# microsoft/Cream

Measured on AMD Instinct MI355X. Metric: images/sec (whole node) AutoFormer-S supernet step @224^2, higher is better.
Workload: dtype bf16; 1 GPU; AutoFormer-S supernet train step, random-path sampling (random.seed(epoch)), per-GPU batch 128, 224x224, AdamW, grad all-reduce RCCL; global_batch=128, parallelism=dp1, wgrad_partials=bf16 split-K partial tiles (within 1.9e-3 of fp32 partials), mixup=on-device, in the timed region

## Files before the change

### cream_amd/_lib.py

```python
import ctypes
import os

_HERE = os.path.dirname(os.path.abspath(__file__))
LIB_PATH = os.path.join(_HERE, "libcream_amd.so")

CREAM_OK = 0
_ERRORS = {
    -1: "CREAM_ERR_BAD_ARG (null pointer, negative size or unsupported stride)",
    -2: "CREAM_ERR_BAD_DTYPE (element type not supported by this entry point)",
    -3: "CREAM_ERR_LAUNCH (HIP kernel launch failed)",
    -4: "CREAM_ERR_TOO_LARGE (shape exceeds what the kernel family supports)",
}

F32, F16, BF16, F64 = 0, 1, 2, 3


class CreamLibraryError(RuntimeError):
    pass


_c = ctypes
_vp, _i, _i64, _f = _c.c_void_p, _c.c_int, _c.c_int64, _c.c_float

SIGNATURES = {
# ... 18 lines not shown
    "cream_irpe_attn2_check": (_i, [_vp, _i]),
    "cream_irpe_attn2_fwd": (_i, [_vp, _vp]),
    "cream_irpe_attn2_bwd": (_i, [_vp, _vp]),
    "cream_irpe_table_grad2": (_i, [_vp, _vp, _i64, _i64, _i64, _i, _vp, _i64, _i64, _i64, _i, _i, _i, _i, _f, _vp]),
    "cream_mini_attn_fwd": (_i, [_vp, _vp]),
    "cream_mini_attn_bwd": (_i, [_vp, _vp]),
    "cream_window_attn_check": (_i, [_vp, _i]),
    "cream_window_attn_part_size": (_i, [_i, _i, _i]),
    "cream_window_attn_blocks": (_i, [_vp]),
    "cream_window_attn_fwd": (_i, [_vp, _vp]),
    "cream_window_attn_bwd": (_i, [_vp, _vp]),
    "cream_window_attn_large_check": (_i, [_vp, _i]),
    "cream_window_attn_large_part_size": (_i, [_i, _i]),
    "cream_window_attn_large_blocks": (_i, [_vp]),
    "cream_window_attn_large_fwd": (_i, [_vp, _vp]),
    "cream_window_attn_large_bwd": (_i, [_vp, _vp]),
    "cream_token_dwconv3_part_size": (_i, [_i]),
    "cream_token_dwconv3_blocks": (_i, [_vp]),
    "cream_token_dwconv3_fwd": (_i, [_vp, _vp]),
    "cream_token_dwconv3_bwd": (_i, [_vp, _vp]),
    "cream_cga_attn_check": (_i, [_vp]),
    "cream_cga_attn_fwd": (_i, [_vp, _vp]),
    "cream_relation_loss_check": (_i, [_vp]),
    "cream_relation_loss_blocks": (_i, [_vp]),
    "cream_relation_loss": (_i, [_vp, _vp]),
    "cream_hidden_relation_check": (_i, [_vp]),
    "cream_hidden_relation_padded": (_i, [_i]),
    "cream_hidden_relation_parts": (_i, [_i, _i]),
    "cream_hidden_relation_loss": (_i, [_vp, _vp]),
    "cream_attn_rpe2d_padded_len": (_i, [_i]),
    "cream_attn_rpe2d_dtab_parts": (_i, [_i, _i]),
    "cream_attn_rpe2d_bwd_mode": (_i, [_i]),
    "cream_attn_rpe2d_fwd": (_i, [_vp, _vp, _vp, _vp, _vp, _vp, _i64, _i64, _i64, _vp, _vp, _vp, _vp, _i,
                                  _i, _i, _i, _i, _i, _i, _f, _i, _vp]),
    "cream_attn_rpe2d_bwd": (_i, [_vp, _vp, _vp, _i64, _i64, _i64, _vp, _vp, _vp, _vp, _vp,
                                  _vp, _vp, _vp, _vp, _vp, _vp, _vp, _i64, _i64, _i64,
                                  _vp, _vp, _vp, _vp, _i, _i, _i, _i, _i, _i, _i, _f, _i, _vp]),
    "cream_attn_rpe2d_fwd_img": (_i, [_vp, _vp, _vp, _vp, _vp, _vp, _i64, _i64, _i64, _vp, _vp, _vp, _vp, _i, _vp,
                                      _i, _i, _i, _i, _i, _i, _f, _i, _vp]),
    "cream_attn_rpe2d_bwd_img": (_i, [_vp, _vp, _vp, _i64, _i64, _i64, _vp, _vp, _vp, _vp, _vp,
                                      _vp, _vp, _vp, _vp, _vp, _vp, _vp, _i64, _i64, _i64,
                                      _vp, _vp, _vp, _vp, _i, _vp, _i, _i, _i, _i, _i, _i, _f, _i, _vp]),
    "cream_attn_rpe2d_fwd_drop": (_i, [_vp, _vp, _vp, _vp, _vp, _vp, _i64, _i64, _i64, _vp, _vp, _vp, _vp, _i, _vp,
                                       _i, _i, _i, _i, _i, _i, _f, _f, _c.c_uint32, _i, _vp]),
    "cream_attn_rpe2d_bwd_drop": (_i, [_vp, _vp, _vp, _i64, _i64, _i64, _vp, _vp, _vp, _vp, _vp,
                                       _vp, _vp, _vp, _vp, _vp, _vp, _vp, _i64, _i64, _i64,
                                       _vp, _vp, _vp, _vp, _i, _vp, _i, _i, _i, _i, _i, _i, _f, _f, _c.c_uint32, _i, _vp]),
    "cream_attn_rpe2d_table_image_bytes": (_i64, []),
    "cream_attn_rpe2d_table_images": (_i, [_vp, _vp, _vp, _vp, _vp, _i, _i, _vp]),
    "cream_attn_rpe2d_fwd_mode": (_i, [_i]),
    "cream_ln_fwd": (_i, [_vp, _vp, _vp, _vp, _vp, _vp, _i, _i, _f, _vp]),
    "cream_ln_partials": (_i, []),
    "cream_ln_bwd": (_i, [_vp, _vp, _vp, _vp, _vp, _vp, _vp, _vp, _vp, _vp, _i, _i, _i, _vp]),
    "cream_gelu_fwd": (_i, [_vp, _vp, _i64, _vp]),
    "cream_gelu_bwd": (_i, [_vp, _vp, _vp, _i64, _vp]),
    "cream_residual_add": (_i, [_vp, _vp, _vp, _vp, _i64, _i64, _vp]),
    "cream_scale_cast": (_i, [_vp, _vp, _vp, _i64, _i64, _vp]),
    "cream_colsum_slabs": (_i, [_i]),
    "cream_colsum": (_i, [_vp, _vp, _i, _i, _vp]),
    "cream_add_ln_fwd": (_i, [_vp, _vp, _vp, _vp, _vp, _vp, _vp, _i, _vp, _vp, _i, _i, _f, _vp]),
    "cream_block_wgrad_bf16": (_i, [_i]),
    "cream_colsum128_slabs": (_i, [_i]),
    "cream_colsum128": (_i, [_vp, _vp, _i, _i, _vp]),
    "cream_gelu_bwd_colsum": (_i, [_vp, _vp, _vp, _vp, _i, _i, _vp]),
    "cream_scale_cast_colsum": (_i, [_vp, _vp, _vp, _vp, _i, _i, _i, _vp]),
    "cream_grad_finalize": (_i, [_vp, _i, _vp]),
    "cream_gemm_rows_per_colsum_slab": (_i, []),
    "cream_gemm_nt256": (_i, [_i]),
    "cream_gemm_nt8": (_i, [_i]),
    "cream_linear_fwd": (_i, [_vp, _vp, _vp, _vp, _i, _i, _i, _i64, _vp]),
    "cream_linear_fwd_seg": (_i, [_vp, _vp, _vp, _vp, _i, _i, _i, _i64, _i, _i64, _vp]),
    "cream_linear_gelu_fwd": (_i, [_vp, _vp, _vp, _vp, _vp, _i, _i, _i, _i64, _vp]),
    "cream_linear_gelu_fwd_pad": (_i, [_vp, _vp, _vp, _vp, _vp, _i, _i, _i, _i, _i64, _vp]),
    "cream_linear_dgrad": (_i, [_vp, _vp, _vp, _i, _i, _i, _i64, _vp]),
    "cream_linear_dgrad_seg": (_i, [_vp, _vp, _vp, _i, _i, _i, _i64, _i, _i64, _vp]),
    "cream_linear_dgrad_mul": (_i, [_vp, _vp, _vp, _vp, _vp, _i, _i, _i, _i64, _vp]),
    "cream_linear_wgrad_splits": (_i, [_i, _i, _i]),
    "cream_linear_wgrad_splits_bf16": (_i, [_i, _i, _i]),
    "cream_gemm_tn8": (_i, [_i]),
    "cream_gemm_nthalf": (_i, [_i]),
    "cream_gemm_nt224": (_i, [_i]),
    "cream_gemm_nt224_launches": (_i64, []),
    "cream_linear_nt224": (_i, [_vp, _vp, _vp, _vp, _i, _i, _i, _i64, _i, _i64, _i, _i64, _vp]),
    "cream_gemm_ntopt": (_i, [_i]),
    "cream_gemm_stagger": (_i, [_i]),
    "cream_block_layout_epoch": (_i, []),
    "cream_cu_reserve": (_i, [_i]),
    "cream_mixup_cutmix": (_i, [_vp, _vp, _vp, _i, _i, _i, _i, _i, _f, _i, _i, _i, _i, _i, _f, _vp]),
    "cream_image_batch_plan": (_i64, [_vp, _i, _i, _i]),
    "cream_image_batch_transform": (_i, [_vp, _vp, _i64, _vp, _vp, _i, _i, _i, _vp, _vp, _vp, _i64, _vp]),
    "cream_cu_count": (_i, []),
    "cream_linear_wgrad_parts": (_i, [_vp, _vp, _vp, _vp, _i, _i, _i, _i, _vp]),
    "cream_linear_wgrad_parts_bf16": (_i, [_vp, _vp, _vp, _vp, _i, _i, _i, _i, _vp]),
    "cream_param_job_tiles": (_i, [_i, _i]),
    "cream_adamw_step": (_i, [_vp, _vp, _i, _i, _i, _c.c_double, _c.c_double, _c.c_double, _c.c_double, _i64, _vp]),
    "cream_grad_clip_coef": (_i, [_vp, _vp, _i, _i, _c.c_double, _vp, _vp, _vp]),
    "cream_adamw_step_clipped": (_i, [_vp, _vp, _i, _i, _i, _c.c_double, _c.c_double, _c.c_double, _c.c_double, _i64, _vp, _vp]),
    "cream_grad_scale": (_i, [_vp, _vp, _i, _i, _vp, _vp]),
    "cream_soft_ce": (_i, [_vp, _vp, _vp, _vp, _i, _i, _i, _f, _vp]),
    "cream_sparse_ce": (_i, [_vp, _vp, _vp, _vp, _vp, _i, _i, _i, _i, _f, _vp]),
    "cream_softmax_topk_records": (_i, [_vp, _vp, _vp, _i, _i, _i, _i, _vp]),
    "cream_linear_f32_fwd": (_i, [_vp, _vp, _vp, _vp, _i, _i, _i, _i64, _i64, _i, _i, _vp]),
    "cream_bmm_f32": (_i, [_vp, _vp, _vp, _i, _i, _i, _vp, _vp, _vp, _i, _i, _vp]),
    "cream_linear_f32_dgrad": (_i, [_vp, _vp, _vp, _i, _i, _i, _i64, _i, _i, _vp]),
    "cream_linear_f32_wgrad": (_i, [_vp, _vp, _vp, _vp, _i, _i, _i, _i64, _i64, _i, _i, _vp]),
    "cream_ln_f32_fwd": (_i, [_vp, _vp, _vp, _vp, _vp, _vp, _i, _i, _f, _vp]),
    "cream_ln_f32_bwd": (_i, [_vp, _vp, _vp, _vp, _vp, _vp, _vp, _i, _i, _vp]),
    "cream_block_prof_enable": (_i, [_i]),
    "cream_block_prof_kinds": (_i, []),
    "cream_block_prof_name": (_c.c_char_p, [_i]),
    "cream_block_prof_collect": (_i, [_vp, _vp, _vp, _vp]),
    "cream_slices_copy": (_i, [_vp, _i, _vp, _i, _i, _vp]),
    "cream_block_fwd_workspace": (_i64, [_vp, _vp, _vp, _vp]),
    "cream_block_fwd": (_i, [_vp, _vp, _vp, _vp, _vp, _vp, _vp]),
    "cream_block_bwd_workspace": (_i64, [_vp, _vp, _vp, _vp]),
    "cream_block_bwd": (_i, [_vp, _vp, _vp, _vp, _vp, _vp, _vp, _vp, _i, _i64, _vp, _vp, _i, _vp, _vp]),
    "cream_image_augment_workspace": (_i64, [_i, _i, _i, _i]),
    "cream_image_augment_u8": (_i, [_vp, _vp, _i, _i, _i, _vp, _vp, _i, _vp, _i64, _vp]),
    "cream_image_batch_plan_aug": (_i64, [_vp, _i, _i, _i, _vp, _i]),
    "cream_image_batch_transform_aug": (_i, [_vp, _vp, _i64, _vp, _vp, _i, _i, _i, _vp, _vp, _vp, _vp, _i, _vp, _i64, _vp]),
}

MAX_GRAD_JOBS = 24


class GradJob(ctypes.Structure):
    _fields_ = [("dst", _vp), ("src", _vp), ("ld", _i64), ("pstride", _i64),
                ("nparts", _c.c_int32), ("rows", _c.c_int32), ("cols", _c.c_int32),
                ("interleave", _c.c_int32), ("src_bf16", _c.c_int32), ("overwrite", _c.c_int32)]

class ImageDesc(ctypes.Structure):
    _fields_ = ([("offset", _i64)] +
                [(n, _c.c_int32) for n in ("height", "width", "row_stride", "box_top", "box_left", "box_h", "box_w", "resized_h",
                                           "resized_w", "win_top", "win_left", "flip", "row0", "nrows")] +
                [("tmp_off", _i64)] +
                [(n, _c.c_int32) for n in ("erase_top", "erase_left", "erase_h", "erase_w")] +
                [("erase_seed", _c.c_uint32), ("reserved", _c.c_int32)])


class AugOp(ctypes.Structure):
    _fields_ = [("kind", _c.c_int32), ("arg", _c.c_int32), ("factor", _f), ("fill", _c.c_uint32), ("m", _c.c_double * 6)]


class SliceJob(ctypes.Structure):
    _fields_ = [("full", _vp), ("ld", _i64), ("packed_off", _i64), ("rows", _c.c_int32), ("cols", _c.c_int32)]


class BlockDesc(ctypes.Structure):
    _fields_ = ([(n, _c.c_int32) for n in ("B", "N", "E", "H", "F", "gh", "gw", "mr", "F_valid", "inference")] +
                [(n, _f) for n in ("eps1", "eps2", "attn_scale", "reserved_f")] +
                [(n, _vp) for n in ("wqkv", "wqkv_t", "bqkv", "wproj", "wproj_t", "bproj", "w1", "w1_t", "b1",
                                    "w2", "w2_t", "b2")] +
                [(n, _i64) for n in ("ld_qkv", "ld_qkv_t", "seg_qkv", "seg_qkv_t", "ld_proj", "ld_proj_t", "ld_w1",
                                     "ld_w1_t", "ld_w2", "ld_w2_t")] +
                [(n, _vp) for n in ("ln1_g", "ln1_b", "ln2_g", "ln2_b", "tkv", "tkh", "tvv", "tvh")] +
                [("ldt", _i64), ("timg", _vp)])


class IrpeAttnDesc(ctypes.Structure):
    _fields_ = ([(n, _vp) for n in ("q", "k", "v")] + [(n, _i64) for n in ("sb", "sn", "sh")] +
                [(n, _vp) for n in ("out", "lse", "sv", "wq", "wk", "wv")] +
                [(n, _i64) for n in ("wq_hs", "wk_hs", "wv_hs")] +
                [(n, _vp) for n in ("idq", "idk", "idv", "idq_t", "idk_t", "idv_t")] +
                [(n, _c.c_int32) for n in ("B", "H", "L", "NP", "nb")] + [("scale", _f)] +
                [(n, _vp) for n in ("dout", "dq", "dk", "dv")] + [(n, _i64) for n in ("dsb", "dsn", "dsh")] +
                [(n, _vp) for n in ("delta", "lkg", "gg", "dlk", "dlq", "bq", "bk")] + [(n, _i64) for n in ("bq_hs", "bk_hs")] +
# ... 128 lines not shown
```

### cream_amd/csrc/gemm_mfma.hip

```cpp
#include <hip/hip_runtime.h>
#include <stdint.h>
#include <stdlib.h>
#include <atomic>

#include "cream_amd.h"
#include "gemm_mfma.hpp"
#include "gemm_nt8.hpp"
#include "gemm_nt224.hpp"
#include "gemm_tn8.hpp"
#include "launch_ev.hpp"
#include "cu_budget.hpp"
#include "env_switch.hpp"

namespace {
std::atomic<int> g_cu_reserve{0};
std::atomic<int> g_layout_epoch{0};
int physical_cus()
{
    static int cus = 0;
    if (!cus) {
        int dev = 0;
        hipDeviceProp_t prop;
        if (hipGetDevice(&dev) == hipSuccess && hipGetDeviceProperties(&prop, dev) == hipSuccess) cus = prop.multiProcessorCount;
        if (cus <= 0) cus = 256;
    }
    return cus;
}
}
namespace cream {
int cu_count()
{
    int c = (physical_cus() - g_cu_reserve.load(std::memory_order_relaxed)) / 8 * 8;
    return c < 8 ? 8 : c;
}
}

namespace {
using namespace cream;
using namespace cream::gemm;

int num_cus() { return cream::cu_count(); }

EnvSwitch g_nt256{"CREAM_GEMM_NT256", 2};
int nt256_mode() { return g_nt256.get(); }

EnvSwitch g_ntopt{"CREAM_GEMM_NTOPT", 3, [](int m) { return m & 15; }};
int ntopt_mode() { return g_ntopt.get(); }
EnvSwitch g_stagger{"CREAM_GEMM_STAGGER", 0};
int stagger_mode() { return g_stagger.get(); }

template <int EPI>
int launch_nt256(const NtParams& p, hipStream_t st)
{
    constexpr int BM = 256, BN = 256;
    auto kern = (ntopt_mode() & 4) ? gemm_nt_kernel<BM, BN, 2, 4, 2, EPI, 1, 1> : gemm_nt_kernel<BM, BN, 2, 4, 2, EPI, 1>;
    constexpr int lds = nt_lds_bytes(BM, BN, 2);
    if (!cream::raise_dynamic_lds(kern, lds)) return CREAM_ERR_LAUNCH;
    const int tiles = ((p.M + BM - 1) / BM) * ((p.N + BN - 1) / BN), slots = num_cus() / 8 * 8;
    CREAM_LAUNCH(kern, dim3(tiles < slots ? tiles : slots), dim3(512), lds, st, p);
    return hipGetLastError() == hipSuccess ? CREAM_OK : CREAM_ERR_LAUNCH;
}

EnvSwitch g_nt8{"CREAM_GEMM_NT8", 4};
int nt8_mode() { return g_nt8.get(); }

bool nt8_fits(const NtParams& p)
{
    const int64_t amax = (int64_t)p.M * p.lda, bmax = (int64_t)2 * p.nseg_stride + (int64_t)p.nseg * p.ldb + p.ldb;
    const int64_t bplain = (int64_t)p.N * p.ldb;
    return amax < ((int64_t)1 << 31) && bmax < ((int64_t)1 << 31) && bplain < ((int64_t)1 << 31) && p.lda < (1 << 24) && p.ldb < (1 << 24);
}

template <int EPI>
int launch_nt8(const NtParams& p, hipStream_t st)
{
    auto kern = gemm_nt8_kernel<EPI>;
    if (!cream::raise_dynamic_lds(kern, NT8_LDS_BYTES)) return CREAM_ERR_LAUNCH;
    const int slots = num_cus() / 8 * 8;
    const int tiles = ((p.M + 255) / 256) * ((p.N + 255) / 256);
    CREAM_LAUNCH(kern, dim3(tiles < slots ? tiles : slots), dim3(512), NT8_LDS_BYTES, st, p);
    return hipGetLastError() == hipSuccess ? CREAM_OK : CREAM_ERR_LAUNCH;
}

EnvSwitch g_nthalf{"CREAM_GEMM_NTHALF", 1, norm_bool};
int nthalf_mode() { return g_nthalf.get(); }

template <int EPI, int BN, int WM, int WN>
int launch_nt_half(const NtParams& p, hipStream_t st)
{
    constexpr int BM = 256;
    auto kern = (ntopt_mode() & 4) ? gemm_nt_kernel<BM, BN, WM, WN, 2, EPI, 1, 1> : gemm_nt_kernel<BM, BN, WM, WN, 2, EPI, 1>;
    constexpr int lds = nt_lds_bytes(BM, BN, 2);
    if (!cream::raise_dynamic_lds(kern, lds)) return CREAM_ERR_LAUNCH;
    const int tiles = ((p.M + BM - 1) / BM) * ((p.N + BN - 1) / BN), slots = num_cus() / 8 * 8;
    CREAM_LAUNCH(kern, dim3(tiles < slots ? tiles : slots), dim3(WM * WN * 64), lds, st, p);
    return hipGetLastError() == hipSuccess ? CREAM_OK : CREAM_ERR_LAUNCH;
}

EnvSwitch g_nt224{"CREAM_GEMM_NT224", 1, norm_bool};
int nt224_mode() { return g_nt224.get(); }
std::atomic<int64_t> g_nt224_launches{0};

template <int EPI>
int launch_nt224(const NtParams& p, hipStream_t st)
{
    auto kern = gemm_nt224_kernel<EPI>;
    if (!cream::raise_dynamic_lds(kern, NT224_LDS_BYTES)) return CREAM_ERR_LAUNCH;
    const int tiles = ((p.M + NT224_BM - 1) / NT224_BM) * ((p.N + NT224_BN - 1) / NT224_BN), slots = num_cus() / 8 * 8;
    CREAM_LAUNCH(kern, dim3(tiles < slots ? tiles : slots), dim3(512), NT224_LDS_BYTES, st, p);
    g_nt224_launches.fetch_add(1, std::memory_order_relaxed);
    return hipGetLastError() == hipSuccess ? CREAM_OK : CREAM_ERR_LAUNCH;
}

template <int EPI>
int launch_nt(const NtParams& p, hipStream_t st)
{
    if constexpr (EPI == EPI_STORE || EPI == EPI_BIAS) {
        if (nt224_mode() > 0 && p.M >= 1024) {
            if (p.N == 448) return launch_nt224<EPI>(p, st);
            if (EPI == EPI_BIAS && p.N == 1344 && p.nseg == 448) return launch_nt224<EPI>(p, st);
        }
        if (nthalf_mode() > 0 && p.M >= 1024) {
            if (p.N == 384 || p.N == 320) return launch_nt_half<EPI, 192, 4, 2>(p, st);
        }
    }
    {
        const int m8 = nt8_mode();
        const bool light = EPI == EPI_STORE || EPI == EPI_BIAS;
        const int npad = (p.N + 255) / 256 * 256;
        if ((m8 == 1 || (m8 == 2 && (light || p.K >= 1024)) || (m8 == 3 && light && (npad - p.N) * 8 <= npad) ||
             (m8 == 4 && EPI == EPI_BIAS && (npad - p.N) * 8 <= npad) ||
             (m8 == 4 && p.K >= 640 && p.N >= 640)) && nt8_fits(p))
            return launch_nt8<EPI>(p, st);
    }
    {
        const int m256 = nt256_mode();
        if ((m256 == 1 && p.N >= 960) || (m256 == 2 && p.K >= 1152) || (m256 == 3 && p.K >= 960)) return launch_nt256<EPI>(p, st);
    }
    const int mode_ = ntopt_mode();
    const bool bwd_epi = EPI == EPI_MUL_COLSUM || EPI == EPI_STORE;
    const int opt = (bwd_epi && !(mode_ & 8)) ? 0 : mode_;
    if (p.N >= 640) {
        constexpr int BM = 128, BN = 128, OCC = 2;
        const int tiles = ((p.M + BM - 1) / BM) * ((p.N + BN - 1) / BN), slots = OCC * num_cus() / 8 * 8;
        NtParams q = p;
        q.stagger = tiles > slots / 2 ? stagger_mode() : 0;
        if (EPI == EPI_BIAS_GELU && (opt & 3) == 3) {
            auto kern = gemm_nt_kernel<BM, BN, 2, 2, 2, EPI, OCC, 3>;
            constexpr int lds = nt_lds_bytes(BM, BN, 2) + GELU_TAB_BYTES;
            if (!cream::raise_dynamic_lds(kern, lds)) return CREAM_ERR_LAUNCH;
            CREAM_LAUNCH(kern, dim3(tiles < slots ? tiles : slots), dim3(256), lds, st, q);
        } else if (opt & 1) {
            CREAM_LAUNCH((gemm_nt_kernel<BM, BN, 2, 2, 2, EPI, OCC, 1>), dim3(tiles < slots ? tiles : slots), dim3(256), 0, st, q);
        } else {
            CREAM_LAUNCH((gemm_nt_kernel<BM, BN, 2, 2, 2, EPI, OCC>), dim3(tiles < slots ? tiles : slots), dim3(256), 0, st, q);
        }
    } else {
        constexpr int BM = 128, BN = 64, OCC = 3;
        const int tiles = ((p.M + BM - 1) / BM) * ((p.N + BN - 1) / BN), slots = OCC * num_cus() / 8 * 8;
        if (opt & 1) {
            CREAM_LAUNCH((gemm_nt_kernel<BM, BN, 2, 2, 2, EPI, OCC, 1>), dim3(tiles < slots ? tiles : slots), dim3(256), 0, st, p);
        } else {
            CREAM_LAUNCH((gemm_nt_kernel<BM, BN, 2, 2, 2, EPI, OCC>), dim3(tiles < slots ? tiles : slots), dim3(256), 0, st, p);
        }
    }
    return hipGetLastError() == hipSuccess ? CREAM_OK : CREAM_ERR_LAUNCH;
}

bool aligned16(const void* p) { return ((uintptr_t)p & 15) == 0; }

int check_nt(const void* out, const void* a, const void* b, int M, int N, int K, int64_t ldb, int kmin_ld)
{
    if (M < 0 || N <= 0 || K <= 0 || ldb < kmin_ld) return CREAM_ERR_BAD_ARG;
    if (N % 8 || K % 8 || ldb % 8) return CREAM_ERR_BAD_ARG;
    if (M == 0) return 1;
    if (!out || !a || !b || !aligned16(out) || !aligned16(a) || !aligned16(b)) return CREAM_ERR_BAD_ARG;
    return CREAM_OK;
}

NtParams plain(void* out, const void* a, const void* b, int M, int N, int K, int64_t ldb)
{
    NtParams p{};
    p.A = (const uint16_t*)a; p.lda = K;
    p.B = (const uint16_t*)b; p.ldb = ldb;
    p.nseg = N; p.kseg = K; p.nseg_stride = 0; p.kseg_stride = 0;
    p.M = M; p.N = N; p.K = K;
    p.out = (uint16_t*)out; p.ldo = N;
    return p;
}

}

extern "C" {

int cream_gemm_rows_per_colsum_slab(void) { return 128; }

int cream_gemm_nt256(int on) { return g_nt256.set(on); }
int cream_gemm_nthalf(int on) { return g_nthalf.set(on); }
int cream_gemm_nt224(int on) { return g_nt224.set(on); }
int64_t cream_gemm_nt224_launches(void) { return g_nt224_launches.load(std::memory_order_relaxed); }
int cream_gemm_ntopt(int mode) { return g_ntopt.set(mode); }
int cream_gemm_stagger(int n) { return g_stagger.set(n); }
int cream_gemm_nt8(int mode) { return g_nt8.set(mode); }

int cream_linear_fwd(void* out, const void* x, const void* w, const void* bias, int M, int N, int K, int64_t ldw,
                     void* stream)
{
    const int rc = check_nt(out, x, w, M, N, K, ldw, K);
    if (rc) return rc < 0 ? rc : CREAM_OK;
    NtParams p = plain(out, x, w, M, N, K, ldw);
    p.bias = (const uint16_t*)bias;
    return launch_nt<EPI_BIAS>(p, (hipStream_t)stream);
}

int cream_linear_fwd_seg(void* out, const void* x, const void* w, const void* bias, int M, int N, int K, int64_t ldw,
                         int nseg, int64_t nseg_stride, void* stream)
{
    const int rc = check_nt(out, x, w, M, N, K, ldw, K);
    if (rc) return rc < 0 ? rc : CREAM_OK;
    if (nseg <= 0 || nseg % 8 || (int64_t)3 * nseg < N || nseg_stride % 8) return CREAM_ERR_BAD_ARG;
    NtParams p = plain(out, x, w, M, N, K, ldw);
    p.bias = (const uint16_t*)bias;
    p.nseg = nseg; p.nseg_stride = nseg_stride;
    return launch_nt<EPI_BIAS>(p, (hipStream_t)stream);
}

int cream_linear_nt224(void* out, const void* x, const void* w, const void* bias, int M, int N, int K, int64_t ldw, int nseg,
                       int64_t nseg_stride, int kseg, int64_t kseg_stride, void* stream)
{
    const int rc = check_nt(out, x, w, M, N, K, ldw, kseg > 0 && kseg < K ? kseg : K);
    if (rc) return rc < 0 ? rc : CREAM_OK;
    NtParams p = plain(out, x, w, M, N, K, ldw);
    if (nseg > 0) {
        if (nseg % 8 || (int64_t)3 * nseg < N || nseg_stride % 8) return CREAM_ERR_BAD_ARG;
        p.nseg = nseg; p.nseg_stride = nseg_stride;
    }
    if (kseg > 0) {
        if (kseg % 64 || K % kseg || kseg_stride % 8) return CREAM_ERR_BAD_ARG;
        p.kseg = kseg; p.kseg_stride = kseg_stride;
    }
    p.bias = (const uint16_t*)bias;
    return bias ? launch_nt224<EPI_BIAS>(p, (hipStream_t)stream) : launch_nt224<EPI_STORE>(p, (hipStream_t)stream);
}

int cream_linear_gelu_fwd_pad(void* gp, void* g, const void* x, const void* w, const void* bias, int M, int N, int Nvalid,
                              int K, int64_t ldw, void* stream)
{
    const int rc = check_nt(gp ? gp : g, x, w, M, N, K, ldw, K);
    if (rc) return rc < 0 ? rc : CREAM_OK;
    if (!g || !bias || !aligned16(g) || Nvalid <= 0 || Nvalid > N) return CREAM_ERR_BAD_ARG;
    NtParams p = plain(gp, x, w, M, N, K, ldw);
    p.bias = (const uint16_t*)bias;
    p.out2 = (uint16_t*)g;
    p.nvalid = Nvalid;
    return launch_nt<EPI_BIAS_GELU>(p, (hipStream_t)stream);
}

int cream_linear_gelu_fwd(void* gp, void* g, const void* x, const void* w, const void* bias, int M, int N, int K,
                          int64_t ldw, void* stream)
{
    return cream_linear_gelu_fwd_pad(gp, g, x, w, bias, M, N, N, K, ldw, stream);
}

int cream_linear_dgrad(void* dx, const void* dy, const void* wt, int M, int N, int K, int64_t ldwt, void* stream)
{
    const int rc = check_nt(dx, dy, wt, M, K, N, ldwt, N);
    if (rc) return rc < 0 ? rc : CREAM_OK;
    const NtParams p = plain(dx, dy, wt, M, K, N, ldwt);
    return launch_nt<EPI_STORE>(p, (hipStream_t)stream);
}

int cream_linear_dgrad_seg(void* dx, const void* dy, const void* wt, int M, int N, int K, int64_t ldwt, int kseg,
                           int64_t kseg_stride, void* stream)
{
    const int rc = check_nt(dx, dy, wt, M, K, N, ldwt, kseg);
    if (rc) return rc < 0 ? rc : CREAM_OK;
    if (kseg <= 0 || kseg % 64 || N % kseg || kseg_stride % 8) return CREAM_ERR_BAD_ARG;
    NtParams p = plain(dx, dy, wt, M, K, N, ldwt);
    p.kseg = kseg; p.kseg_stride = kseg_stride;
    return launch_nt<EPI_STORE>(p, (hipStream_t)stream);
}

int cream_linear_dgrad_mul(void* dh, float* colsum_parts, const void* dy, const void* wt, const void* factor, int M, int N,
                             int K, int64_t ldwt, void* stream)
{
    const int rc = check_nt(dh, dy, wt, M, K, N, ldwt, N);
    if (rc) return rc < 0 ? rc : CREAM_OK;
    if (!colsum_parts || !factor || !aligned16(factor)) return CREAM_ERR_BAD_ARG;
    NtParams p = plain(dh, dy, wt, M, K, N, ldwt);
    p.aux = (const uint16_t*)factor; p.ldaux = K;
    p.colsum = colsum_parts;
    return launch_nt<EPI_MUL_COLSUM>(p, (hipStream_t)stream);
}

}

namespace {
EnvSwitch g_tn8{"CREAM_GEMM_TN8", 2};
int tn8_mode() { return g_tn8.get(); }
int tn8_tiles(int N, int K) { return ((N + 255) / 256) * ((K + 255) / 256); }
int tn8_splits(int M, int N, int K)
{
    const int T = tn8_tiles(N, K), steps = (M + 63) / 64;
    static const int share = getenv("CREAM_WGRAD_CUS") ? atoi(getenv("CREAM_WGRAD_CUS")) : 0;
    int slots = num_cus() / 2 / 8 * 8;
    if (share >= 8) slots = (share < num_cus() ? share : num_cus()) / 8 * 8;
    int s = slots / T;
    if (s > steps) s = steps;
    return s < 1 ? 1 : s;
}
bool tn8_wanted(int M, int N, int K)
{
    const int mode = tn8_mode();
    if (mode <= 0 || M <= 0 || N % 8 || K % 8) return false;
    const int T = tn8_tiles(N, K);
    if ((int64_t)64 * (N > K ? N : K) * 2 + 4096 >= ((int64_t)1 << 31)) return false;
    return mode >= 2 ? T <= num_cus() : (T >= 6 && T <= num_cus());
}
}

extern "C" {

int cream_gemm_tn8(int mode)
{
    const int prev = g_tn8.set(mode);
// ... 81 lines not shown
```

### cream_amd/csrc/gemm_nt224.hpp

```cpp
#pragma once
#include "gemm_mfma.hpp"

namespace cream {
namespace gemm {

constexpr int NT224_BM = 256, NT224_BN = 224;
constexpr int NT224_LDS_BYTES = nt_lds_bytes(NT224_BM, NT224_BN, 2);

template <int EPI>
__global__ __launch_bounds__(512, 2) void gemm_nt224_kernel(const NtParams p)
{
    static_assert(EPI == EPI_STORE || EPI == EPI_BIAS, "plain and bias epilogues only");
    constexpr int BM = NT224_BM, BN = NT224_BN, BK = 64;
    constexpr int WN = 2, NW = 8, NT = NW * 64;
    constexpr int WTM = 64, WTN = 112, TM = WTM / 16, TN = WTN / 16;
    constexpr int STAGE = (BM + BN) * BK;
    constexpr int PIECES = (BM + BN) / 8;
    constexpr int NPIECE = (PIECES + NW - 1) / NW;
    constexpr int APIECE = BM / 8 / NW;
    constexpr int NCH = BN / 4;
    constexpr int HM = 64, NPASS = BM / HM;
    static_assert(PIECES % NW != 0 && HM == WTM && HM * BN * 4 <= STAGE * 2, "tile");
    char* const smem = LdsBlock<NT224_LDS_BYTES>::get();
    uint16_t* const lds = reinterpret_cast<uint16_t*>(smem);
    float* const ctile = reinterpret_cast<float*>(smem + STAGE * 2);

    const int tid = threadIdx.x, lane = tid & 63, q = lane >> 4, l15 = lane & 15;
    const int wave = __builtin_amdgcn_readfirstlane(tid >> 6);
    const int wm = wave / WN, wn = wave % WN;
    const int ntn = (p.N + BN - 1) / BN, ntiles = ntn * ((p.M + BM - 1) / BM);
    const int K = p.K;

    const int prow = wave * 8 + (lane >> 3);
    const int cch = ((lane & 7) ^ ((prow >> 1) & 7)) * 8;
    auto sources = [&](const uint16_t* (&src)[NPIECE], int m0, int n0) {
#pragma unroll
        for (int i = 0; i < NPIECE; ++i) {
            const int row = prow + NW * 8 * i;
            if (i < APIECE) {
                src[i] = p.A + (int64_t)min(m0 + row, p.M - 1) * p.lda + cch;
            } else {
                const int n = min(n0 + min(row - BM, BN - 1), p.N - 1);
                const int seg = (n >= p.nseg) + (n >= 2 * p.nseg);
                src[i] = p.B + seg * p.nseg_stride + (int64_t)(n - seg * p.nseg) * p.ldb + cch;
            }
        }
    };
    int64_t kb = 0;
    int kin = 0;
    auto issue = [&](const uint16_t* const (&src)[NPIECE], int k0, int buf, auto tail) {
#pragma unroll
        for (int i = 0; i < NPIECE; ++i) {
            if (i == NPIECE - 1 && wave + NW * i >= PIECES) continue;
            const uint16_t* s = src[i] + (i < APIECE ? (int64_t)k0 : kb);
            if constexpr (decltype(tail)::value) s += min(0, K - 8 - (k0 + cch));
            __builtin_amdgcn_global_load_lds(
                s, reinterpret_cast<__attribute__((address_space(3))) void*>(
                       reinterpret_cast<uintptr_t>(lds + buf * STAGE + (wave + NW * i) * 8 * BK)), 16, 0, 0);
        }
        kb += BK;
        kin += BK;
        if (kin >= p.kseg) { kin = 0; kb += p.kseg_stride - p.kseg; }
    };
    const int sw = l15 >> 1;
    auto frag = [&](const uint16_t* tile, int row, int chunk) -> bf16x8 {
        return *reinterpret_cast<const bf16x8*>(tile + row * BK + ((chunk ^ sw) << 3));
    };

    f32x4v acc[TN][TM];

    auto step = [&](int buf, int vc, auto tail) {
        constexpr bool T = decltype(tail)::value;
        const uint16_t* At = lds + buf * STAGE + (wm * WTM + l15) * BK;
        const uint16_t* Bt = lds + buf * STAGE + (BM + wn * WTN + l15) * BK;
        const bf16x8 zero = bf16x8{0, 0, 0, 0, 0, 0, 0, 0};
        bf16x8 fa[2][TM], fb[2 * TN];
        auto ra = [&](int ks, int i) {
            fa[ks][i] = frag(At, i * 16, ks * 4 + q);
            if (T && ks * 4 + q >= vc) fa[ks][i] = zero;
        };
        auto rb = [&](int j) {
            const int ks = j / TN;
            fb[j] = frag(Bt, (j % TN) * 16, ks * 4 + q);
            if (T && ks * 4 + q >= vc) fb[j] = zero;
        };
#pragma unroll
        for (int i = 0; i < TM; ++i) ra(0, i);
#pragma unroll
        for (int j = 0; j < 2 * TN; ++j) {
            rb(j);
            if (j == 5) { ra(1, 0); ra(1, 1); }
            if (j == 7) { ra(1, 2); ra(1, 3); }
        }
#pragma unroll
        for (int j = 0; j < 2 * TN; ++j) {
#pragma unroll
            for (int tm = 0; tm < TM; ++tm)
                acc[j % TN][tm] = __builtin_amdgcn_mfma_f32_16x16x32_bf16(fb[j], fa[j / TN][tm], acc[j % TN][tm], 0, 0, 0);
        }
        {
            __builtin_amdgcn_sched_group_barrier(0x100, TM + 2, 0);
#pragma unroll
            for (int u = 0; u < TN; ++u) {
                __builtin_amdgcn_sched_group_barrier(0x008, 1, 0);
                if (u == 1 || u == 2) __builtin_amdgcn_sched_group_barrier(0x100, 4, 0);
                else if (u + 1 < TN) __builtin_amdgcn_sched_group_barrier(0x100, 2, 0);
                __builtin_amdgcn_sched_group_barrier(0x008, 2 * TM - 1, 0);
            }
        }
    };
    using No = std::integral_constant<bool, false>;
    using Yes = std::integral_constant<bool, true>;
    const int nfull = K / BK, rem = K % BK, nk = nfull + (rem ? 1 : 0);

    constexpr int CPR = BN / 8;
    constexpr int RPP = NT / CPR;
    constexpr int NJ = (HM + RPP - 1) / RPP;
    const int cc = tid % CPR, r0 = tid / CPR;
    const bool epi_thread = tid < CPR * RPP;
    static_assert(NCH % 8 == 0, "XOR inside groups of 8 positions");
    const int wpos = wn * (WTN / 8) + (q >> 1) + (NCH / 2) * (q & 1);

    int orig = blockIdx.x;
    const uint16_t* src[NPIECE];
    int t = xcd_remap(orig, ntiles);
    int m0 = (t / ntn) * BM, n0 = (t % ntn) * BN;
    sources(src, m0, n0);
    if (0 < nfull) issue(src, 0, 0, No{}); else issue(src, 0, 0, Yes{});

    for (;;) {
#pragma unroll
        for (int a = 0; a < TN; ++a)
#pragma unroll
            for (int b = 0; b < TM; ++b) acc[a][b] = f32x4v{0, 0, 0, 0};

        auto top_of_step = [&](int s) {
            wait_vmcnt<0>();
            __builtin_amdgcn_s_barrier();
            asm volatile("" ::: "memory");
            if (s + 1 < nk) { if (s + 1 < nfull) issue(src, (s + 1) * BK, (s + 1) & 1, No{}); else issue(src, (s + 1) * BK, (s + 1) & 1, Yes{}); }
        };
        for (int s = 0; s < nfull; ++s) {
            top_of_step(s);
            step(s & 1, 8, No{});
        }
        if (rem) {
            top_of_step(nfull);
            step(nfull & 1, rem >> 3, Yes{});
        }

        const int n = n0 + cc * 8;
        const bool ncol_ok = n < p.N && epi_thread;
        const int cur_m0 = m0;
        const int next = orig + (int)gridDim.x;
        const bool has_next = next < ntiles;
        __syncthreads();
        if (has_next) {
            orig = next;
            t = xcd_remap(orig, ntiles);
            m0 = (t / ntn) * BM; n0 = (t % ntn) * BN;
            sources(src, m0, n0);
            kb = 0; kin = 0;
            if (0 < nfull) issue(src, 0, 0, No{}); else issue(src, 0, 0, Yes{});
        }

        u32x4v braw = u32x4v{0, 0, 0, 0};
        if constexpr (EPI == EPI_BIAS) {
            if (p.bias && ncol_ok) braw = *reinterpret_cast<const u32x4v*>(p.bias + n);
        }
        float bv[8];
#pragma unroll
        for (int e = 0; e < 4; ++e) {
            bv[2 * e] = __uint_as_float(braw[e] << 16);
            bv[2 * e + 1] = __uint_as_float(braw[e] & 0xFFFF0000u);
        }
#pragma unroll
        for (int pass = 0; pass < NPASS; ++pass) {
            if (pass) __syncthreads();
            if (wm == pass) {
#pragma unroll
                for (int tn = 0; tn < TN; ++tn)
#pragma unroll
                    for (int tm = 0; tm < TM; ++tm) {
                        const int ml = tm * 16 + l15;
                        *reinterpret_cast<f32x4v*>(ctile + ml * BN + (((wpos + 2 * tn) ^ (l15 & 7)) << 2)) = acc[tn][tm];
                    }
            }
            __syncthreads();
#pragma unroll
            for (int j = 0; j < NJ; ++j) {
                const int row = r0 + j * RPP, m = cur_m0 + pass * HM + row;
                if (row >= HM || m >= p.M || !ncol_ok) continue;
                const f32x4v lo = *reinterpret_cast<const f32x4v*>(ctile + row * BN + ((cc ^ (row & 7)) << 2));
                const f32x4v hi = *reinterpret_cast<const f32x4v*>(ctile + row * BN + (((cc + NCH / 2) ^ (row & 7)) << 2));
                float v[8] = {lo[0], lo[1], lo[2], lo[3], hi[0], hi[1], hi[2], hi[3]};
#pragma unroll
                for (int e = 0; e < 8; ++e) v[e] += bv[e];
                st_out16(p.out + (int64_t)m * p.ldo + n,
                         u32x4v{f2bf_pair(v[0], v[1]), f2bf_pair(v[2], v[3]), f2bf_pair(v[4], v[5]), f2bf_pair(v[6], v[7])});
            }
        }
        if (!has_next) break;
    }
}

}
}
```

### include/cream_amd.h

```cpp
#ifndef CREAM_AMD_H_
#define CREAM_AMD_H_

#include <stdint.h>

#ifdef __cplusplus
extern "C" {
#endif

#define CREAM_OK               0
#define CREAM_ERR_BAD_ARG     -1
#define CREAM_ERR_BAD_DTYPE   -2
#define CREAM_ERR_LAUNCH      -3
#define CREAM_ERR_TOO_LARGE   -4

#define CREAM_F32   0
#define CREAM_F16   1
#define CREAM_BF16  2
#define CREAM_F64   3

const char* cream_version(void);

const char* cream_build_info(void);


// ... 251 lines not shown
    float* part;
    void *dq, *dk, *dv;
    int64_t dsb, dsn;
} cream_relation_desc;

int cream_relation_loss_check(const cream_relation_desc* d);

int cream_relation_loss_blocks(const cream_relation_desc* d);

int cream_relation_loss(const cream_relation_desc* d, void* stream);

typedef struct cream_hidden_relation_desc {
    const void *s, *t;
    int32_t s_dtype, t_dtype, B, L, Cs, Ct, want_grad;
    float coef;
    void *sn, *tn;
    float *s_rinv, *t_rinv, *g, *part;
    void* ds;
} cream_hidden_relation_desc;

int cream_hidden_relation_check(const cream_hidden_relation_desc* d);
int cream_hidden_relation_padded(int C);
int cream_hidden_relation_parts(int B, int L);
int cream_hidden_relation_loss(const cream_hidden_relation_desc* d, void* stream);

typedef struct cream_irpe_attn2_desc {
    cream_irpe_attn_desc base;
    int32_t head_dim;
    int32_t row_width;
    const uint8_t* key_pad;
    int64_t key_pad_sb;
    int64_t osb, osn, dosb, dosn;
} cream_irpe_attn2_desc;

int cream_irpe_attn2_check(const cream_irpe_attn2_desc* d, int backward);

int cream_irpe_attn2_fwd(const cream_irpe_attn2_desc* d, void* stream);

int cream_irpe_attn2_bwd(const cream_irpe_attn2_desc* d, void* stream);

int cream_irpe_table_grad2(float* out, const void* x, int64_t xsb, int64_t xsn, int64_t xsh, int xa, const void* y,
                           int64_t ysb, int64_t ysn, int64_t ysh, int yc, int B, int H, int L, float mul, void* stream);


int cream_ln_fwd(void* y, float* mean, float* rstd, const float* x, const float* gamma,
                 const float* beta, int M, int E, float eps, void* stream);

int cream_add_ln_fwd(float* xsum, void* y, float* mean, float* rstd, const float* x, const void* res,
                     const float* sample_scale, int rows_per_sample, const float* gamma,
                     const float* beta, int M, int E, float eps, void* stream);

int cream_ln_partials(void);

int cream_ln_bwd(float* dx, void* dx_scaled, float* partial, const void* dy, const float* x,
                 const float* mean, const float* rstd, const float* gamma, const float* dres,
                 const float* sample_scale, int rows_per_sample, int M, int E, void* stream);

int cream_gelu_fwd(void* g, const void* h, int64_t n, void* stream);
int cream_gelu_bwd(void* dh, const void* dg, const void* h, int64_t n, void* stream);

int cream_residual_add(float* out, const float* x, const void* y, const float* sample_scale,
                       int64_t n, int64_t per_sample, void* stream);

int cream_scale_cast(void* out, const float* x, const float* sample_scale, int64_t n,
                     int64_t per_sample, void* stream);

int cream_colsum_slabs(int M);
int cream_colsum(float* partial, const void* a, int M, int C, void* stream);

int cream_colsum128_slabs(int M);
int cream_colsum128(float* partial, const void* a, int M, int C, void* stream);
int cream_gelu_bwd_colsum(void* dh, float* partial, const void* dg, const void* h, int M, int C,
                          void* stream);
int cream_scale_cast_colsum(void* out, float* partial, const float* x, const float* sample_scale,
                            int rows_per_sample, int M, int C, void* stream);

int cream_gemm_rows_per_colsum_slab(void);

int cream_gemm_nt256(int on);
int cream_gemm_nthalf(int on);
int cream_gemm_nt224(int on);
int64_t cream_gemm_nt224_launches(void);
int cream_linear_nt224(void* out, const void* x, const void* w, const void* bias, int M, int N, int K, int64_t ldw, int nseg,
                       int64_t nseg_stride, int kseg, int64_t kseg_stride, void* stream);
int cream_gemm_nt8(int mode);
int cream_gemm_ntopt(int mode);
int cream_gemm_stagger(int n);
int cream_linear_fwd(void* out, const void* x, const void* w, const void* bias, int M, int N, int K,
                     int64_t ldw, void* stream);
int cream_linear_fwd_seg(void* out, const void* x, const void* w, const void* bias, int M, int N, int K,
                         int64_t ldw, int nseg, int64_t nseg_stride, void* stream);
int cream_linear_gelu_fwd(void* gp, void* g, const void* x, const void* w, const void* bias, int M, int N,
                          int K, int64_t ldw, void* stream);
int cream_linear_gelu_fwd_pad(void* gp, void* g, const void* x, const void* w, const void* bias, int M, int N, int Nvalid,
                              int K, int64_t ldw, void* stream);
int cream_linear_dgrad(void* dx, const void* dy, const void* wt, int M, int N, int K, int64_t ldwt,
                       void* stream);
int cream_linear_dgrad_seg(void* dx, const void* dy, const void* wt, int M, int N, int K, int64_t ldwt,
                           int kseg, int64_t kseg_stride, void* stream);
int cream_linear_dgrad_mul(void* dh, float* colsum_parts, const void* dy, const void* wt, const void* factor,
                             int M, int N, int K, int64_t ldwt, void* stream);
int cream_linear_wgrad_splits(int M, int N, int K);
int cream_linear_wgrad_parts(float* parts, float* bias_parts, const void* dy, const void* x, int M, int N,
                             int K, int S, void* stream);
int cream_linear_wgrad_parts_bf16(void* parts_bf16, float* bias_parts, const void* dy, const void* x, int M, int N,
                                  int K, int S, void* stream);
int cream_linear_wgrad_splits_bf16(int M, int N, int K);
int cream_gemm_tn8(int mode);

typedef struct cream_param_job {
    float* p;
    const float* g;
    float *m, *v;
    void *mir, *mir_t;
    int64_t ld, ld_mir, ld_mir_t, seg_stride, seg_stride_t;
    int32_t rows, cols, deinterleave;
    float weight_decay;
} cream_param_job;
int cream_param_job_tiles(int rows, int cols);
int cream_adamw_step(const cream_param_job* jobs_dev, const int32_t* first_tile_dev, int njobs, int total_tiles,
                     int update, double lr, double beta1, double beta2, double eps, int64_t step, void* stream);

int cream_grad_clip_coef(const cream_param_job* jobs_dev, const int32_t* first_tile_dev, int njobs, int total_tiles,
                         double max_norm, double* partials_dev, float* out_dev, void* stream);
int cream_adamw_step_clipped(const cream_param_job* jobs_dev, const int32_t* first_tile_dev, int njobs, int total_tiles,
                             int update, double lr, double beta1, double beta2, double eps, int64_t step,
                             const float* coef_dev, void* stream);
int cream_grad_scale(const cream_param_job* jobs_dev, const int32_t* first_tile_dev, int njobs, int total_tiles,
                     const float* coef_dev, void* stream);

typedef struct cream_grad_job {
    float* dst;
    const void* src;
    int64_t ld;
    int64_t pstride;
    int32_t nparts, rows, cols;
    int32_t interleave;
    int32_t src_bf16;
    int32_t overwrite;
} cream_grad_job;
#define CREAM_MAX_GRAD_JOBS 24
int cream_grad_finalize(const cream_grad_job* jobs, int njobs, void* stream);

typedef struct cream_image_desc {
    int64_t offset;
    int32_t height, width, row_stride;
    int32_t box_top, box_left, box_h, box_w;
    int32_t resized_h, resized_w;
    int32_t win_top, win_left;
    int32_t flip;
    int32_t row0, nrows;
    int64_t tmp_off;
    int32_t erase_top, erase_left, erase_h, erase_w;
    uint32_t erase_seed;
    int32_t reserved;
} cream_image_desc;
int64_t cream_image_batch_plan(cream_image_desc* descs, int B, int out_h, int out_w);
int cream_image_batch_transform(float* out, const uint8_t* pixels, int64_t pixels_bytes, const cream_image_desc* descs,
                                const cream_image_desc* descs_dev, int B, int out_h, int out_w, const float* mean,
                                const float* stdev, void* workspace, int64_t workspace_bytes, void* stream);

int cream_mixup_cutmix(float* x, float* y, const int64_t* target, int B, int Cimg, int H, int W, int num_classes, float lam,
                       int use_cutmix, int yl, int yh, int xl, int xh, float label_smoothing, void* stream);

int cream_soft_ce(float* loss_rows, float* dlogits, const void* logits, const float* target, int B, int C, int logits_dtype,
                  float grad_scale, void* stream);
// ... 112 lines not shown
```

Before: 14970 images/sec.

## Generalize nt224 GEMM kernel to BN=160 with three-stage pipelining

Templates the 256x224 NT GEMM kernel on column tile width and adds a 256x160 variant, used by default for N=320 forward GEMMs in place of the 192-wide half-tile kernel. When a third LDS stage fits in the budget (the BN=160 case), the kernel prefetches two K-steps ahead and waits on a partial vmcnt, overlapping loads with MFMA. The intent is to avoid the padding waste of 192-wide tiles on N=320 and to hide more global-load latency. The cost is a larger LDS footprint, which may limit occupancy, and a more complex schedule.

```diff
diff --git a/cream_amd/_lib.py b/cream_amd/_lib.py
--- a/cream_amd/_lib.py
+++ b/cream_amd/_lib.py
@@ -124,6 +124,9 @@
     "cream_gemm_nt224": (_i, [_i]),
     "cream_gemm_nt224_launches": (_i64, []),
     "cream_linear_nt224": (_i, [_vp, _vp, _vp, _vp, _i, _i, _i, _i64, _i, _i64, _i, _i64, _vp]),
+    "cream_gemm_nt160": (_i, [_i]),
+    "cream_gemm_nt160_launches": (_i64, []),
+    "cream_linear_nt160": (_i, [_vp, _vp, _vp, _vp, _i, _i, _i, _i64, _i, _i64, _i, _i64, _vp]),
     "cream_gemm_ntopt": (_i, [_i]),
     "cream_gemm_stagger": (_i, [_i]),
     "cream_block_layout_epoch": (_i, []),
diff --git a/cream_amd/csrc/gemm_mfma.hip b/cream_amd/csrc/gemm_mfma.hip
--- a/cream_amd/csrc/gemm_mfma.hip
+++ b/cream_amd/csrc/gemm_mfma.hip
@@ -101,16 +101,27 @@
 int nt224_mode() { return g_nt224.get(); }
 std::atomic<int64_t> g_nt224_launches{0};
 
+template <int EPI, int BN>
+int launch_nt16(const NtParams& p, hipStream_t st, std::atomic<int64_t>& launches)
+{
+    auto kern = gemm_nt16_kernel<EPI, BN>;
+    constexpr int lds = nt16_lds_bytes(BN);
+    if (!cream::raise_dynamic_lds(kern, lds)) return CREAM_ERR_LAUNCH;
+    const int tiles = ((p.M + NT16_BM - 1) / NT16_BM) * ((p.N + BN - 1) / BN), slots = num_cus() / 8 * 8;
+    CREAM_LAUNCH(kern, dim3(tiles < slots ? tiles : slots), dim3(512), lds, st, p);
+    launches.fetch_add(1, std::memory_order_relaxed);
+    return hipGetLastError() == hipSuccess ? CREAM_OK : CREAM_ERR_LAUNCH;
+}
+
 template <int EPI>
-int launch_nt224(const NtParams& p, hipStream_t st)
-{
-    auto kern = gemm_nt224_kernel<EPI>;
-    if (!cream::raise_dynamic_lds(kern, NT224_LDS_BYTES)) return CREAM_ERR_LAUNCH;
-    const int tiles = ((p.M + NT224_BM - 1) / NT224_BM) * ((p.N + NT224_BN - 1) / NT224_BN), slots = num_cus() / 8 * 8;
-    CREAM_LAUNCH(kern, dim3(tiles < slots ? tiles : slots), dim3(512), NT224_LDS_BYTES, st, p);
-    g_nt224_launches.fetch_add(1, std::memory_order_relaxed);
-    return hipGetLastError() == hipSuccess ? CREAM_OK : CREAM_ERR_LAUNCH;
-}
+int launch_nt224(const NtParams& p, hipStream_t st) { return launch_nt16<EPI, 224>(p, st, g_nt224_launches); }
+
+EnvSwitch g_nt160{"CREAM_GEMM_NT160", 1, norm_bool};
+int nt160_mode() { return g_nt160.get(); }
+std::atomic<int64_t> g_nt160_launches{0};
+
+template <int EPI>
+int launch_nt160(const NtParams& p, hipStream_t st) { return launch_nt16<EPI, 160>(p, st, g_nt160_launches); }
 
 template <int EPI>
 int launch_nt(const NtParams& p, hipStream_t st)
@@ -119,6 +130,9 @@
         if (nt224_mode() > 0 && p.M >= 1024) {
             if (p.N == 448) return launch_nt224<EPI>(p, st);
             if (EPI == EPI_BIAS && p.N == 1344 && p.nseg == 448) return launch_nt224<EPI>(p, st);
+        }
+        if (nt160_mode() > 0 && p.M >= 1024) {
+            if (p.N == 320) return launch_nt160<EPI>(p, st);
         }
         if (nthalf_mode() > 0 && p.M >= 1024) {
             if (p.N == 384 || p.N == 320) return launch_nt_half<EPI, 192, 4, 2>(p, st);
@@ -189,6 +203,24 @@
     return p;
 }
 
+int direct_nt(NtParams& p, void* out, const void* x, const void* w, const void* bias, int M, int N, int K, int64_t ldw, int nseg,
+              int64_t nseg_stride, int kseg, int64_t kseg_stride)
+{
+    const int rc = check_nt(out, x, w, M, N, K, ldw, kseg > 0 && kseg < K ? kseg : K);
+    if (rc) return rc;
+    p = plain(out, x, w, M, N, K, ldw);
+    if (nseg > 0) {
+        if (nseg % 8 || (int64_t)3 * nseg < N || nseg_stride % 8) return CREAM_ERR_BAD_ARG;
+        p.nseg = nseg; p.nseg_stride = nseg_stride;
+    }
+    if (kseg > 0) {
+        if (kseg % 64 || K % kseg || kseg_stride % 8) return CREAM_ERR_BAD_ARG;
+        p.kseg = kseg; p.kseg_stride = kseg_stride;
+    }
+    p.bias = (const uint16_t*)bias;
+    return CREAM_OK;
+}
+
 }
 
 extern "C" {
@@ -199,6 +231,8 @@
 int cream_gemm_nthalf(int on) { return g_nthalf.set(on); }
 int cream_gemm_nt224(int on) { return g_nt224.set(on); }
 int64_t cream_gemm_nt224_launches(void) { return g_nt224_launches.load(std::memory_order_relaxed); }
+int cream_gemm_nt160(int on) { return g_nt160.set(on); }
+int64_t cream_gemm_nt160_launches(void) { return g_nt160_launches.load(std::memory_order_relaxed); }
 int cream_gemm_ntopt(int mode) { return g_ntopt.set(mode); }
 int cream_gemm_stagger(int n) { return g_stagger.set(n); }
 int cream_gemm_nt8(int mode) { return g_nt8.set(mode); }
@@ -228,19 +262,19 @@
 int cream_linear_nt224(void* out, const void* x, const void* w, const void* bias, int M, int N, int K, int64_t ldw, int nseg,
                        int64_t nseg_stride, int kseg, int64_t kseg_stride, void* stream)
 {
-    const int rc = check_nt(out, x, w, M, N, K, ldw, kseg > 0 && kseg < K ? kseg : K);
-    if (rc) return rc < 0 ? rc : CREAM_OK;
-    NtParams p = plain(out, x, w, M, N, K, ldw);
-    if (nseg > 0) {
-        if (nseg % 8 || (int64_t)3 * nseg < N || nseg_stride % 8) return CREAM_ERR_BAD_ARG;
-        p.nseg = nseg; p.nseg_stride = nseg_stride;
-    }
-    if (kseg > 0) {
-        if (kseg % 64 || K % kseg || kseg_stride % 8) return CREAM_ERR_BAD_ARG;
-        p.kseg = kseg; p.kseg_stride = kseg_stride;
-    }
-    p.bias = (const uint16_t*)bias;
+    NtParams p{};
+    const int rc = direct_nt(p, out, x, w, bias, M, N, K, ldw, nseg, nseg_stride, kseg, kseg_stride);
+    if (rc) return rc < 0 ? rc : CREAM_OK;
     return bias ? launch_nt224<EPI_BIAS>(p, (hipStream_t)stream) : launch_nt224<EPI_STORE>(p, (hipStream_t)stream);
+}
+
+int cream_linear_nt160(void* out, const void* x, const void* w, const void* bias, int M, int N, int K, int64_t ldw, int nseg,
+                       int64_t nseg_stride, int kseg, int64_t kseg_stride, void* stream)
+{
+    NtParams p{};
+    const int rc = direct_nt(p, out, x, w, bias, M, N, K, ldw, nseg, nseg_stride, kseg, kseg_stride);
+    if (rc) return rc < 0 ? rc : CREAM_OK;
+    return bias ? launch_nt160<EPI_BIAS>(p, (hipStream_t)stream) : launch_nt160<EPI_STORE>(p, (hipStream_t)stream);
 }
 
 int cream_linear_gelu_fwd_pad(void* gp, void* g, const void* x, const void* w, const void* bias, int M, int N, int Nvalid,
diff --git a/cream_amd/csrc/gemm_nt224.hpp b/cream_amd/csrc/gemm_nt224.hpp
--- a/cream_amd/csrc/gemm_nt224.hpp
+++ b/cream_amd/csrc/gemm_nt224.hpp
@@ -4,26 +4,30 @@
 namespace cream {
 namespace gemm {
 
-constexpr int NT224_BM = 256, NT224_BN = 224;
-constexpr int NT224_LDS_BYTES = nt_lds_bytes(NT224_BM, NT224_BN, 2);
-
-template <int EPI>
-__global__ __launch_bounds__(512, 2) void gemm_nt224_kernel(const NtParams p)
+constexpr int NT16_BM = 256;
+constexpr int nt16_stages(int BN) { return nt_lds_bytes(NT16_BM, BN, 3) <= 160 * 1024 ? 3 : 2; }
+constexpr int nt16_lds_bytes(int BN) { return nt_lds_bytes(NT16_BM, BN, nt16_stages(BN)); }
+
+template <int EPI, int BN>
+__global__ __launch_bounds__(512, 2) void gemm_nt16_kernel(const NtParams p)
 {
     static_assert(EPI == EPI_STORE || EPI == EPI_BIAS, "plain and bias epilogues only");
-    constexpr int BM = NT224_BM, BN = NT224_BN, BK = 64;
+    static_assert(BN == 224 || BN == 160, "column tiles of 2 x 7 and 2 x 5 blocks");
+    constexpr int BM = NT16_BM, BK = 64;
     constexpr int WN = 2, NW = 8, NT = NW * 64;
-    constexpr int WTM = 64, WTN = 112, TM = WTM / 16, TN = WTN / 16;
+    constexpr int WTM = 64, WTN = BN / WN, TM = WTM / 16, TN = WTN / 16;
+    static_assert(WTN % 16 == 0 && TN % 2 == 1 && TN >= 5, "an odd number of blocks per wave column: see the schedule in `step`");
     constexpr int STAGE = (BM + BN) * BK;
+    constexpr int NST = nt16_stages(BN), D = NST - 1;
     constexpr int PIECES = (BM + BN) / 8;
     constexpr int NPIECE = (PIECES + NW - 1) / NW;
     constexpr int APIECE = BM / 8 / NW;
     constexpr int NCH = BN / 4;
     constexpr int HM = 64, NPASS = BM / HM;
-    static_assert(PIECES % NW != 0 && HM == WTM && HM * BN * 4 <= STAGE * 2, "tile");
-    char* const smem = LdsBlock<NT224_LDS_BYTES>::get();
+    static_assert(PIECES % NW != 0 && HM == WTM && HM * BN * 4 <= STAGE * 2 && (D == 1 || D == 2), "tile");
+    char* const smem = LdsBlock<nt16_lds_bytes(BN)>::get();
     uint16_t* const lds = reinterpret_cast<uint16_t*>(smem);
-    float* const ctile = reinterpret_cast<float*>(smem + STAGE * 2);
+    float* const ctile = reinterpret_cast<float*>(smem + D * STAGE * 2);
 
     const int tid = threadIdx.x, lane = tid & 63, q = lane >> 4, l15 = lane & 15;
     const int wave = __builtin_amdgcn_readfirstlane(tid >> 6);
@@ -89,8 +93,8 @@
 #pragma unroll
         for (int j = 0; j < 2 * TN; ++j) {
             rb(j);
-            if (j == 5) { ra(1, 0); ra(1, 1); }
-            if (j == 7) { ra(1, 2); ra(1, 3); }
+            if (j == TN - 2) { ra(1, 0); ra(1, 1); }
+            if (j == TN) { ra(1, 2); ra(1, 3); }
         }
 #pragma unroll
         for (int j = 0; j < 2 * TN; ++j) {
@@ -103,7 +107,7 @@
 #pragma unroll
             for (int u = 0; u < TN; ++u) {
                 __builtin_amdgcn_sched_group_barrier(0x008, 1, 0);
-                if (u == 1 || u == 2) __builtin_amdgcn_sched_group_barrier(0x100, 4, 0);
+                if (u == (TN - 5) / 2 || u == (TN - 3) / 2) __builtin_amdgcn_sched_group_barrier(0x100, 4, 0);
                 else if (u + 1 < TN) __builtin_amdgcn_sched_group_barrier(0x100, 2, 0);
                 __builtin_amdgcn_sched_group_barrier(0x008, 2 * TM - 1, 0);
             }
@@ -118,7 +122,7 @@
     constexpr int NJ = (HM + RPP - 1) / RPP;
     const int cc = tid % CPR, r0 = tid / CPR;
     const bool epi_thread = tid < CPR * RPP;
-    static_assert(NCH % 8 == 0, "XOR inside groups of 8 positions");
+    static_assert(NCH % 8 == 0 && WTN % 8 == 0, "XOR inside groups of 8 positions; a wave column starts on an even chunk");
     const int wpos = wn * (WTN / 8) + (q >> 1) + (NCH / 2) * (q & 1);
 
     int orig = blockIdx.x;
@@ -126,7 +130,13 @@
     int t = xcd_remap(orig, ntiles);
     int m0 = (t / ntn) * BM, n0 = (t % ntn) * BN;
     sources(src, m0, n0);
-    if (0 < nfull) issue(src, 0, 0, No{}); else issue(src, 0, 0, Yes{});
+    auto issue_step = [&](int s, int buf) { if (s < nfull) issue(src, s * BK, buf, No{}); else issue(src, s * BK, buf, Yes{}); };
+    auto stage_of = [](int s) { return NST == 2 ? (s & 1) : (int)((unsigned)s % (unsigned)NST); };
+    auto first_steps = [&]() {
+        issue_step(0, 0);
+        if constexpr (D == 2) { if (1 < nk) issue_step(1, 1); }
+    };
+    first_steps();
 
     for (;;) {
 #pragma unroll
@@ -135,18 +145,22 @@
             for (int b = 0; b < TM; ++b) acc[a][b] = f32x4v{0, 0, 0, 0};
 
         auto top_of_step = [&](int s) {
-            wait_vmcnt<0>();
+            if constexpr (D == 2) {
+                if (s > 0 && s + 1 < nk) wait_vmcnt<NPIECE - 1>(); else wait_vmcnt<0>();
+            } else {
+                wait_vmcnt<0>();
+            }
             __builtin_amdgcn_s_barrier();
             asm volatile("" ::: "memory");
-            if (s + 1 < nk) { if (s + 1 < nfull) issue(src, (s + 1) * BK, (s + 1) & 1, No{}); else issue(src, (s + 1) * BK, (s + 1) & 1, Yes{}); }
+            if (s + D < nk) issue_step(s + D, stage_of(s + D));
         };
         for (int s = 0; s < nfull; ++s) {
             top_of_step(s);
-            step(s & 1, 8, No{});
+            step(stage_of(s), 8, No{});
         }
         if (rem) {
             top_of_step(nfull);
-            step(nfull & 1, rem >> 3, Yes{});
+            step(stage_of(nfull), rem >> 3, Yes{});
         }
 
         const int n = n0 + cc * 8;
@@ -161,7 +175,7 @@
             m0 = (t / ntn) * BM; n0 = (t % ntn) * BN;
             sources(src, m0, n0);
             kb = 0; kin = 0;
-            if (0 < nfull) issue(src, 0, 0, No{}); else issue(src, 0, 0, Yes{});
+            first_steps();
         }
 
         u32x4v braw = u32x4v{0, 0, 0, 0};
diff --git a/include/cream_amd.h b/include/cream_amd.h
--- a/include/cream_amd.h
+++ b/include/cream_amd.h
@@ -357,6 +357,10 @@
 int cream_gemm_nt224(int on);
 int64_t cream_gemm_nt224_launches(void);
 int cream_linear_nt224(void* out, const void* x, const void* w, const void* bias, int M, int N, int K, int64_t ldw, int nseg,
+                       int64_t nseg_stride, int kseg, int64_t kseg_stride, void* stream);
+int cream_gemm_nt160(int on);
+int64_t cream_gemm_nt160_launches(void);
+int cream_linear_nt160(void* out, const void* x, const void* w, const void* bias, int M, int N, int K, int64_t ldw, int nseg,
                        int64_t nseg_stride, int kseg, int64_t kseg_stride, void* stream);
 int cream_gemm_nt8(int mode);
 int cream_gemm_ntopt(int mode);
```

After: 15090 images/sec, median of 6. About the same (+0.8%).
